# leejaehot/GaussianGrasper

Hardware: AMD Instinct MI355X
Metric: rendered views/sec (fwd+bwd) at 1M Gaussians, 1600x1200, 32-ch feature (higher is better)
Workload: dtype f32; 1 GPU; BASELINE config 4 per-GPU share: 1000000 Gaussians, 1600x1200, SH deg 4 rgb + 32-ch feature + depth + normal images per view (nerfstudio plugin route: the timed callable is FusedGaussianSplattingModel.get_outputs(camera) of gaussiangrasper_amd.plugin (the class train.sh loads, on stub.py's stand-ins for nerfstudio's base model and Cameras) — one fused rasterize operator per view), fwd+bwd, 8 views; route=plugin, deterministic_backward=False, python_gc=gc.freeze() after the warm-up (bench.freeze_gc), view_pipeline=backward of view k beside forward of view k + 1 on two streams, num_gaussians=1000000, feature_dim=32, n_visible=992125, parallelism=view-parallel x1, replicated Gaussians, grad_allreduce_bytes=472000000, grad_allreduce=per parameter, overlapped with the last view's backward

## Files before the change

gaussiangrasper_amd/csrc/blend2.hip:

```cpp
#include <type_traits>

#include "blend_launch.h"

#define GRP 4
#define KEEP(x) asm volatile("" ::"v"(x))

#include "blend_measure.h"
#define LIST_CAP 72

template <int NC = 1>
struct WaveListT {
    float4 a[LIST_CAP];
    float4 b[LIST_CAP];
    float4 c[LIST_CAP];
    float4 d[NC >= 2 ? LIST_CAP : 1];
    float4 e[NC >= 3 ? LIST_CAP : 1];
};

struct Seg2 {
    const float *colors;
    const float *background;
    float *out_img;
    int C2, nch2;
};
// ... 3 lines not shown
    return __builtin_amdgcn_mbcnt_hi((uint32_t)(m >> 32), __builtin_amdgcn_mbcnt_lo((uint32_t)m, 0u));
}

template <int CH, bool WIDE, bool REL = false, typename LIST = WaveList>
__device__ __forceinline__ int stage_chunk(LIST &L, int lane, int e, bool valid,
                                           const int g ,
                                           const GRec *__restrict__ rec,
                                           const float *__restrict__ colors, int C, int ch_off, int nch,
                                           float xlo, float xhi, float ylo, float yhi,
                                           const Seg2 *seg2 = nullptr) {
    const float4 ra = reinterpret_cast<const float4 *>(rec + g)[0];
    const float4 rb = reinterpret_cast<const float4 *>(rec + g)[1];
    const bool hit = valid && rec_hits_rect(ra, rb, xlo, xhi, ylo, yhi);
    const uint64_t m = __ballot(hit);
    const int cnt = __builtin_popcountll(m);
    const int pos = GRP + lane_prefix(m);
    if (hit) {
        const float posf = __builtin_bit_cast(float, REL ? lane : e + 1);
        float4 cc = make_float4(0.f, 0.f, 0.f, posf);
        float4 ra2 = ra;
        if (WIDE) {
            cc.x = __builtin_bit_cast(float, g);
            if (seg2) {
                const float *c2 = seg2->colors + (size_t)g * seg2->C2;
                const int n2 = seg2->nch2;
                L.d[pos] = make_float4(c2[0], n2 > 1 ? c2[1] : 0.f, n2 > 2 ? c2[2] : 0.f, n2 > 3 ? c2[3] : 0.f);
                L.e[pos] = make_float4(n2 > 4 ? c2[4] : 0.f, n2 > 5 ? c2[5] : 0.f, n2 > 6 ? c2[6] : 0.f,
                                       n2 > 7 ? c2[7] : 0.f);
            }
        } else {
            const float *col = colors + (size_t)g * C + ch_off;
            cc.x = col[0];
            if (CH > 1 && nch > 1) cc.y = col[1];
            if (CH > 2 && nch > 2) cc.z = col[2];
            if (CH > 3) {
                cc.w = nch > 3 ? col[3] : 0.f;
                float4 dd = make_float4(0.f, 0.f, 0.f, 0.f);
                if (nch > 4) dd.x = col[4];
                if (nch > 5) dd.y = col[5];
                if (nch > 6) dd.z = col[6];
                if (nch > 7) dd.w = col[7];
                L.d[pos] = dd;
                ra2.w = posf;
            }
        }
        L.a[pos] = ra2;
        L.b[pos] = make_float4(rb.x, rb.y, rb.z, __builtin_bit_cast(float, g));
        L.c[pos] = cc;
    }
    if (lane < 2 * GRP) {
        const int q = (lane < GRP) ? lane : (cnt + lane);
        L.a[q] = make_float4(0.f, 0.f, 0.f, 0.f);
        L.b[q] = make_float4(0.f, 0.f, 0.f, __builtin_bit_cast(float, -1));
        L.c[q] = make_float4(0.f, 0.f, 0.f, 0.f);
        if (CH > 3 && !WIDE) L.d[q] = make_float4(0.f, 0.f, 0.f, 0.f);
        if (WIDE && seg2) {
            L.d[q] = make_float4(0.f, 0.f, 0.f, 0.f);
            L.e[q] = make_float4(0.f, 0.f, 0.f, 0.f);
        }
    }
    __builtin_amdgcn_wave_barrier();
    return cnt;
}

#ifndef GG_FWD_WAVES
#define GG_FWD_WAVES 5
#endif
template <int CH, bool WIDE, bool FULL, bool EX = false, int FABL = 0, int NCB = 1>
__global__ __launch_bounds__(64 * GG_WPB_OTHER)
__attribute__((amdgpu_waves_per_eu((WIDE && EX && NCB == 1) ? GG_FWD_WAVES : (NCB == 2 ? (EX ? 4 : 3) : (NCB > 2 ? 2 : 1)))))
void blend2_fwd_kernel(
    int C, int ch_off, int nch, int img_h, int img_w, int tiles_x, int ntiles,
    const int32_t *__restrict__ ids, const int2 *__restrict__ bins, const GRec *__restrict__ rec,
    const float *__restrict__ colors, const float *__restrict__ background,
    float *__restrict__ out_img, float *__restrict__ final_T, int32_t *__restrict__ final_idx,
    int write_final, Seg2 seg2 = Seg2()) {
    constexpr bool N8 = !WIDE && CH > 3;
    static_assert(!EX || WIDE, "the second array rides on the wide kernel");
    static_assert(NCB == 1 || (WIDE && FULL), "several channel blocks: the full wide builds");
    typedef WaveListT<EX ? 3 : (N8 ? 2 : 1)> LIST;
    __shared__ LIST lists[GG_WPB_OTHER];
    int wave;
    const int tile = blend_tile_wave<GG_WPB_OTHER>(blockIdx.x, threadIdx.x, ntiles, wave);
    if (tile < 0) return;
    const int lane = threadIdx.x & 63;
    const int wslot = wave & (GG_WPB_OTHER - 1);
    LIST &L = lists[wslot];
    const int tx = tile % tiles_x, ty = tile / tiles_x;
    const int qx0 = tx * GG_BLOCK + (wave & 1) * 8, qy0 = ty * GG_BLOCK + (wave >> 1) * 8;
    const int j = qx0 + (lane & 7), i = qy0 + (lane >> 3);
    const bool inside = (i < img_h) && (j < img_w);
    const float px = (float)j, py = (float)i;
    const float xlo = (float)qx0, xhi = (float)(qx0 + 7), ylo = (float)qy0, yhi = (float)(qy0 + 7);
    const int2 range = bins[tile];

    STAMP_DECL;
    float T = 1.0f;
    int last = range.x;
    bool done = !inside;
    float acc[WIDE ? 1 : CH];
    float acc2[EX ? 8 : 1];
#pragma unroll
    for (int c = 0; c < (EX ? 8 : 1); ++c) acc2[c] = 0.0f;
    f32x16 acc0[NCB], acc1[NCB];
#pragma unroll
    for (int c = 0; c < (WIDE ? 1 : CH); ++c) acc[c] = 0.0f;
#pragma unroll
    for (int cb = 0; cb < NCB; ++cb)
#pragma unroll
        for (int r = 0; r < 16; ++r) acc0[cb][r] = acc1[cb][r] = 0.0f;
    const int wch = lane & 31, half = lane >> 5;
    const bool wch_ok = FULL || wch < nch;

    STAMP(0);
    for (int base = range.x; base < range.y; base += 64) {
        if (__ballot(!done) == 0ull) break;
        const int e = base + lane;
        const int g_cur = e < range.y ? ids[e] : 0;
        const int cnt = stage_chunk<CH, WIDE, false, LIST>(L, lane, e, e < range.y, g_cur, rec, colors, C,
                                                           ch_off, nch, xlo, xhi, ylo, yhi, EX ? &seg2 : nullptr);
        WALK_STAT(0, min(64, range.y - base));
        STAMP(1);
        STAMP_BATCH();
        constexpr int fabl = FABL;
        if (fabl >= 4) { KEEP(cnt); continue; }
        for (int k = 0; k < cnt; k += GRP) {
            if (k > 0 && __ballot(!done) == 0ull) break;
            WALK_STAT(1, min(GRP, cnt - k));
            constexpr bool LEANF = WIDE && (EX || NCB > 1);
            float4 A[GRP], B[GRP], Cc[GRP], Cd[GRP];
#pragma unroll
            for (int q = 0; q < GRP; ++q) {
                if (LEANF) continue;
                A[q] = L.a[GRP + k + q];
                B[q] = L.b[GRP + k + q];
                Cc[q] = L.c[GRP + k + q];
                if (N8) Cd[q] = L.d[GRP + k + q];
            }
            float colB[GRP / 2][NCB];
            if (WIDE) {
#pragma unroll
                for (int pr = 0; pr < GRP / 2; ++pr) {
                    const int gid = __builtin_bit_cast(int, L.c[GRP + k + 2 * pr + half].x);
#pragma unroll
                    for (int cb = 0; cb < NCB; ++cb)
                        colB[pr][cb] = (wch_ok && fabl < 2) ? colors[(size_t)gid * C + ch_off + 32 * cb + wch] : 0.0f;
                }
            }
            float alpha[GRP];
            bool pass[GRP];
#pragma unroll
            for (int q = 0; q < GRP; ++q) {
                if (LEANF) {
                    A[q] = L.a[GRP + k + q];
                    B[q] = L.b[GRP + k + q];
                }
                const float dx = A[q].x - px, dy = A[q].y - py;
                const float sigma = __builtin_fmaf(
                    0.5f, __builtin_fmaf(B[q].x * dx, dx, (B[q].z * dy) * dy), (B[q].y * dx) * dy);
                alpha[q] = fminf(GG_ALPHA_MAX_FWD, A[q].z * gg_expf_walk(-sigma));
                pass[q] = sigma >= 0.0f && !(alpha[q] < GG_ALPHA_MIN);
                if (LEANF && q == 1) __builtin_amdgcn_sched_barrier(0);
            }
            float vis[GRP];
#pragma unroll
            for (int q = 0; q < GRP; ++q) {
                const float next_T = T * (1.0f - alpha[q]);
                const bool live = pass[q] && !done;
                const bool stop = live && (next_T <= GG_T_EPS);
                const bool blend = live && !stop;
                vis[q] = blend ? alpha[q] * T : 0.0f;
#ifdef GG_WALK_STATS
                {
                    const unsigned long long bm = __ballot(blend), pm = __ballot(pass[q]), lm = __ballot(!done);
                    WALK_STAT(2, bm != 0ull);
                    WALK_STAT(3, __builtin_popcountll(lm));
                    WALK_STAT(4, __builtin_popcountll(pm));
                    WALK_STAT(5, __builtin_popcountll(bm));
                }
#endif
                T = blend ? next_T : T;
                last = blend ? __builtin_bit_cast(int, N8 ? A[q].w : (LEANF ? L.c[GRP + k + q].w : Cc[q].w)) : last;
                done = done || stop;
                if (EX && fabl < 3) {
                    const float4 xd = L.d[GRP + k + q], xe = L.e[GRP + k + q];
                    acc2[0] = __builtin_fmaf(xd.x, vis[q], acc2[0]);
                    acc2[EX ? 1 : 0] = __builtin_fmaf(xd.y, vis[q], acc2[EX ? 1 : 0]);
                    acc2[EX ? 2 : 0] = __builtin_fmaf(xd.z, vis[q], acc2[EX ? 2 : 0]);
                    acc2[EX ? 3 : 0] = __builtin_fmaf(xd.w, vis[q], acc2[EX ? 3 : 0]);
                    acc2[EX ? 4 : 0] = __builtin_fmaf(xe.x, vis[q], acc2[EX ? 4 : 0]);
                    acc2[EX ? 5 : 0] = __builtin_fmaf(xe.y, vis[q], acc2[EX ? 5 : 0]);
                    acc2[EX ? 6 : 0] = __builtin_fmaf(xe.z, vis[q], acc2[EX ? 6 : 0]);
                    acc2[EX ? 7 : 0] = __builtin_fmaf(xe.w, vis[q], acc2[EX ? 7 : 0]);
                }
                if (!WIDE) {
                    acc[0] = __builtin_fmaf(Cc[q].x, vis[q], acc[0]);
                    if (CH > 1) acc[CH > 1 ? 1 : 0] = __builtin_fmaf(Cc[q].y, vis[q], acc[CH > 1 ? 1 : 0]);
                    if (CH > 2) acc[CH > 2 ? 2 : 0] = __builtin_fmaf(Cc[q].z, vis[q], acc[CH > 2 ? 2 : 0]);
                    if (N8) {
                        acc[CH > 3 ? 3 : 0] = __builtin_fmaf(Cc[q].w, vis[q], acc[CH > 3 ? 3 : 0]);
                        acc[CH > 4 ? 4 : 0] = __builtin_fmaf(Cd[q].x, vis[q], acc[CH > 4 ? 4 : 0]);
                        acc[CH > 5 ? 5 : 0] = __builtin_fmaf(Cd[q].y, vis[q], acc[CH > 5 ? 5 : 0]);
                        acc[CH > 6 ? 6 : 0] = __builtin_fmaf(Cd[q].z, vis[q], acc[CH > 6 ? 6 : 0]);
                        acc[CH > 7 ? 7 : 0] = __builtin_fmaf(Cd[q].w, vis[q], acc[CH > 7 ? 7 : 0]);
                    }
                }
            }
            if (WIDE && fabl >= 1) {
#pragma unroll
                for (int q = 0; q < GRP; ++q) KEEP(vis[q]);
#pragma unroll
                for (int pr = 0; pr < GRP / 2; ++pr) KEEP(colB[pr][0]);
            } else if (WIDE) {
#pragma unroll
                for (int pr = 0; pr < GRP / 2; ++pr) {
                    auto r = __builtin_amdgcn_permlane32_swap(
                        __builtin_bit_cast(unsigned, vis[2 * pr]),
                        __builtin_bit_cast(unsigned, vis[2 * pr + 1]), false, false);
#pragma unroll
                    for (int cb = 0; cb < NCB; ++cb) {
                        acc0[cb] = __builtin_amdgcn_mfma_f32_32x32x2f32(__builtin_bit_cast(float, (unsigned)r[0]),
                                                                        colB[pr][cb], acc0[cb], 0, 0, 0);
                        acc1[cb] = __builtin_amdgcn_mfma_f32_32x32x2f32(__builtin_bit_cast(float, (unsigned)r[1]),
                                                                        colB[pr][cb], acc1[cb], 0, 0, 0);
                    }
                }
            }
        }
        __builtin_amdgcn_wave_barrier();
        STAMP(4);
    }
    STAMP(8);
    if (inside && write_final) {
        const size_t p = (size_t)i * img_w + j;
        final_T[p] = T;
        final_idx[p] = last;
    }
    if (EX && inside) {
        float *o2 = seg2.out_img + ((size_t)i * img_w + j) * seg2.C2;
#pragma unroll
        for (int c = 0; c < 8; ++c)
            if (c < seg2.nch2) o2[c] = __builtin_fmaf(T, seg2.background[c], acc2[EX ? c : 0]);
    }
    if (!WIDE) {
        if (inside) {
            float *o = out_img + ((size_t)i * img_w + j) * C + ch_off;
#pragma unroll
            for (int c = 0; c < CH; ++c)
                if (c < nch) o[c] = __builtin_fmaf(T, background[ch_off + c], acc[c]);
        }
    } else if (FULL && (C % 4 == 0) && (ch_off % 4 == 0) && ((reinterpret_cast<uintptr_t>(out_img) & 15) == 0)) {
        float *buf = reinterpret_cast<float *>(&L);
        const int chunk = lane & 7;
        __builtin_amdgcn_wave_barrier();
#pragma unroll
        for (int cb = 0; cb < NCB; ++cb) {
        const int ch_cb = ch_off + 32 * cb;
        const float4 bg4 = *reinterpret_cast<const float4 *>(background + ch_cb + 4 * chunk);
#pragma unroll
        for (int q4 = 0; q4 < 4; ++q4) {
#pragma unroll
            for (int rr = 0; rr < 8; ++rr) {
                const int r = 8 * (q4 & 1) + rr;
                const int pl = (rr & 3) + 8 * (rr >> 2) + 4 * half;
                buf[pl * 32 + wch] = (q4 >> 1) ? acc1[cb][r] : acc0[cb][r];
            }
            __builtin_amdgcn_wave_barrier();
#pragma unroll
            for (int t = 0; t < 2; ++t) {
                const int pl = (lane >> 3) + 8 * t;
                const float4 v = *reinterpret_cast<const float4 *>(buf + pl * 32 + 4 * chunk);
                const int pq = 16 * q4 + pl;
                const float Tp = __shfl(T, pq, 64);
                const int pj = qx0 + (pq & 7), pi = qy0 + (pq >> 3);
                if (pi < img_h && pj < img_w) {
                    typedef float f4v __attribute__((ext_vector_type(4)));
                    const f4v o = {__builtin_fmaf(Tp, bg4.x, v.x), __builtin_fmaf(Tp, bg4.y, v.y),
                                   __builtin_fmaf(Tp, bg4.z, v.z), __builtin_fmaf(Tp, bg4.w, v.w)};
                    f4v *dst = reinterpret_cast<f4v *>(out_img + ((size_t)pi * img_w + pj) * C + ch_cb + 4 * chunk);
                    *dst = o;
                }
            }
            __builtin_amdgcn_wave_barrier();
        }
        }
    } else {
        const float bgc = wch_ok ? background[ch_off + wch] : 0.0f;
#pragma unroll
        for (int blk = 0; blk < 2; ++blk)
#pragma unroll
            for (int r = 0; r < 16; ++r) {
                const int pq = 32 * blk + (r & 3) + 8 * (r >> 2) + 4 * half;
                const float Tp = __shfl(T, pq, 64);
                const int pj = qx0 + (pq & 7), pi = qy0 + (pq >> 3);
                if (pi < img_h && pj < img_w && wch_ok)
                    out_img[((size_t)pi * img_w + pj) * C + ch_off + wch] =
                        __builtin_fmaf(Tp, bgc, blk ? acc1[0][r] : acc0[0][r]);
            }
    }
    STAMP(7);
    STAMP_END();
}

#define FB_SLOTS 32
#define FB_QCAP 100
#ifndef GG_FB_WAVES
#define GG_FB_WAVES 3
#endif
struct __attribute__((aligned(16))) FwdQueue {
    float4 a[FB_QCAP];
    float4 b[FB_QCAP];
};
#define GG_VIS_SCALE 32768.0f
#define GG_VIS_UNSCALE (1.0f / 32768.0f)

__global__ __launch_bounds__(64) __attribute__((amdgpu_waves_per_eu(GG_FB_WAVES))) void blend2_fwd_batch_kernel(
    int C, int img_h, int img_w, int tiles_x, int ntiles, const int32_t *__restrict__ ids,
    const int2 *__restrict__ bins, const GRec *__restrict__ rec, const float *__restrict__ colors,
    const float *__restrict__ background, float *__restrict__ out_img, float *__restrict__ final_T,
    int32_t *__restrict__ final_idx, Seg2 seg2, unsigned bytes1, unsigned bytes2) {
    __shared__ FwdQueue s_q;
    __shared__ __attribute__((aligned(16))) float s_vis[64 * FB_SLOTS];
    int wave;
    const int tile = blend_tile_wave<1>(blockIdx.x, threadIdx.x, ntiles, wave);
    if (tile < 0) return;
    const int lane = threadIdx.x & 63;
    FwdQueue &Q = s_q;
    float *vis_w = s_vis;
    const int tx = tile % tiles_x, ty = tile / tiles_x;
    const int qx0 = tx * GG_BLOCK + (wave & 1) * 8, qy0 = ty * GG_BLOCK + (wave >> 1) * 8;
    const int j = qx0 + (lane & 7), i = qy0 + (lane >> 3);
    const bool inside = (i < img_h) && (j < img_w);
    const float px = (float)j, py = (float)i;
    const int2 range = bins[tile];
    const int sl = lane & 15, q4 = lane >> 4;

    float T = GG_VIS_SCALE;
    int last = range.x;
    bool done = !inside;
    bool alive = true;
    float csc[3];
#pragma unroll
    for (int nb = 0; nb < 3; ++nb) csc[nb] = pow2_scale(0.0f);
    f32x4 acc[4][3];
#pragma unroll
    for (int blk = 0; blk < 4; ++blk)
#pragma unroll
        for (int nb = 0; nb < 3; ++nb) acc[blk][nb] = f32x4{0.0f, 0.0f, 0.0f, 0.0f};
    const bool ch2_ok = sl < seg2.nch2;
    const __amdgpu_buffer_rsrc_t rs1 = __builtin_amdgcn_make_buffer_rsrc(const_cast<float *>(colors), 0, (int)bytes1, 0x00020000);
    const __amdgpu_buffer_rsrc_t rs2 = __builtin_amdgcn_make_buffer_rsrc(const_cast<float *>(seg2.colors), 0, (int)bytes2, 0x00020000);
    const unsigned rowb1 = 4u * (unsigned)C, rowb2 = 4u * (unsigned)seg2.C2;
    const unsigned lane_off1 = 4u * (unsigned)sl, lane_off2 = ch2_ok ? 4u * (unsigned)sl : 0u;

    auto run_batch = [&](const int base, const int n) {
        float cb[3][8];
#pragma unroll
        for (int t = 0; t < 8; ++t) {
            const int s_ = min(8 * q4 + t, n - 1);
            const unsigned gid = (unsigned)__builtin_bit_cast(int, Q.b[base + s_].w);
            const unsigned o1 = __umul24(gid, rowb1) + lane_off1;
            cb[0][t] = __builtin_bit_cast(float, __builtin_amdgcn_raw_buffer_load_b32(rs1, (int)o1, 0, 0));
            cb[1][t] = __builtin_bit_cast(float, __builtin_amdgcn_raw_buffer_load_b32(rs1, (int)o1 + 64, 0, 0));
            const unsigned o2 = __umul24(gid, rowb2) + lane_off2;
            const float c2v = __builtin_bit_cast(float, __builtin_amdgcn_raw_buffer_load_b32(rs2, (int)o2, 0, 0));
            cb[2][t] = ch2_ok ? c2v : 0.0f;
        }
        int nw = 0;
        for (int g = 0; g < n; g += GRP) {
            if (__ballot(!done) == 0ull) { alive = false; break; }
            float vis[GRP];
#pragma unroll
            for (int q = 0; q < GRP; ++q) {
                const float4 A = Q.a[base + g + q], B = Q.b[base + g + q];
                const float dx = A.x - px, dy = A.y - py;
                const float sigma = __builtin_fmaf(
                    0.5f, __builtin_fmaf(B.x * dx, dx, (B.z * dy) * dy), (B.y * dx) * dy);
                const float alpha = fminf(GG_ALPHA_MAX_FWD, A.z * gg_expf_walk(-sigma));
                const bool pass = sigma >= 0.0f && !(alpha < GG_ALPHA_MIN);
                const float next_T = T * (1.0f - alpha);
                const bool live = pass && !done;
                const bool stop = live && (next_T <= GG_T_EPS * GG_VIS_SCALE);
                const bool blend = live && !stop;
                vis[q] = blend ? alpha * T : 0.0f;
                T = blend ? next_T : T;
                last = blend ? __builtin_bit_cast(int, A.w) : last;
                done = done || stop;
                if (q == 1) __builtin_amdgcn_sched_barrier(0);
            }
            *reinterpret_cast<float4 *>(vis_w + lane * FB_SLOTS + ((((g >> 2) ^ lane) & 7) << 2)) =
                make_float4(vis[0], vis[1], vis[2], vis[3]);
            nw = g + GRP;
        }
        for (int g = nw; g < FB_SLOTS; g += GRP)
            *reinterpret_cast<float4 *>(vis_w + lane * FB_SLOTS + ((((g >> 2) ^ lane) & 7) << 2)) =
                make_float4(0.0f, 0.0f, 0.0f, 0.0f);
        __builtin_amdgcn_wave_barrier();
        h16x8 Bh[3], Bl[3];
        float fac[3];
        bool shrink = false;
#pragma unroll
        for (int nb = 0; nb < 3; ++nb) {
            float m = fmaxf(fmaxf(fabsf(cb[nb][0]), fabsf(cb[nb][1])), fabsf(cb[nb][2]));
            m = fmaxf(fmaxf(m, fabsf(cb[nb][3])), fabsf(cb[nb][4]));
            m = fmaxf(fmaxf(m, fabsf(cb[nb][5])), fmaxf(fabsf(cb[nb][6]), fabsf(cb[nb][7])));
            {
                auto r16 = __builtin_amdgcn_permlane16_swap(__builtin_bit_cast(unsigned, m), __builtin_bit_cast(unsigned, m), false, false);
                m = fmaxf(__builtin_bit_cast(float, (unsigned)r16[0]), __builtin_bit_cast(float, (unsigned)r16[1]));
                auto r32 = __builtin_amdgcn_permlane32_swap(__builtin_bit_cast(unsigned, m), __builtin_bit_cast(unsigned, m), false, false);
                m = fmaxf(__builtin_bit_cast(float, (unsigned)r32[0]), __builtin_bit_cast(float, (unsigned)r32[1]));
            }
            const float sb = fminf(csc[nb], pow2_scale(m));
            fac[nb] = sb * pow2_inv(csc[nb]);
            shrink = shrink || sb != csc[nb];
            csc[nb] = sb;
            unsigned h_[4], l_[4];
#pragma unroll
            for (int t = 0; t < 4; ++t) split2h(cb[nb][2 * t] * sb, cb[nb][2 * t + 1] * sb, h_[t], l_[t]);
            Bh[nb] = H8(h_[0], h_[1], h_[2], h_[3]);
            Bl[nb] = H8(l_[0], l_[1], l_[2], l_[3]);
        }
        if (__ballot(shrink) != 0ull) {
#pragma unroll
            for (int blk = 0; blk < 4; ++blk)
#pragma unroll
                for (int nb = 0; nb < 3; ++nb)
#pragma unroll
                    for (int r = 0; r < 4; ++r) acc[blk][nb][r] *= fac[nb];
        }
#pragma unroll
        for (int blk = 0; blk < 4; ++blk) {
            const int P = 16 * blk + sl;
            const float4 v0 = *reinterpret_cast<const float4 *>(vis_w + P * FB_SLOTS + ((((2 * q4) ^ P) & 7) << 2));
            const float4 v1 = *reinterpret_cast<const float4 *>(vis_w + P * FB_SLOTS + ((((2 * q4 + 1) ^ P) & 7) << 2));
            unsigned ah[4], al[4];
            split2h(v0.x, v0.y, ah[0], al[0]);
            split2h(v0.z, v0.w, ah[1], al[1]);
            split2h(v1.x, v1.y, ah[2], al[2]);
            split2h(v1.z, v1.w, ah[3], al[3]);
            const h16x8 Ah = H8(ah[0], ah[1], ah[2], ah[3]), Al = H8(al[0], al[1], al[2], al[3]);
#pragma unroll
            for (int nb = 0; nb < 3; ++nb) {
                acc[blk][nb] = __builtin_amdgcn_mfma_f32_16x16x32_f16(Al, Bl[nb], acc[blk][nb], 0, 0, 0);
                acc[blk][nb] = __builtin_amdgcn_mfma_f32_16x16x32_f16(Al, Bh[nb], acc[blk][nb], 0, 0, 0);
                acc[blk][nb] = __builtin_amdgcn_mfma_f32_16x16x32_f16(Ah, Bl[nb], acc[blk][nb], 0, 0, 0);
                acc[blk][nb] = __builtin_amdgcn_mfma_f32_16x16x32_f16(Ah, Bh[nb], acc[blk][nb], 0, 0, 0);
            }
        }
        __builtin_amdgcn_wave_barrier();
    };

    int qn = 0;
    int g_nxt = (range.x + lane < range.y) ? ids[range.x + lane] : 0;
    for (int cbase = range.x; cbase < range.y; cbase += 64) {
        if (__ballot(!done) == 0ull) { alive = false; break; }
        const int e = cbase + lane;
        const bool valid = e < range.y;
        const int g = g_nxt;
        g_nxt = (e + 64 < range.y) ? ids[e + 64] : 0;
        const float4 ra = reinterpret_cast<const float4 *>(rec + g)[0];
        const float4 rb = reinterpret_cast<const float4 *>(rec + g)[1];
        int qxl = qx0, qyl = qy0;
        asm volatile("" : "+s"(qxl), "+s"(qyl));
        const bool hit = valid && rec_hits_rect(ra, rb, (float)qxl, (float)(qxl + 7), (float)qyl, (float)(qyl + 7));
        const uint64_t m = __ballot(hit);
        if (hit) {
            const int pos = qn + lane_prefix(m);
            Q.a[pos] = make_float4(ra.x, ra.y, ra.z, __builtin_bit_cast(float, e + 1));
            Q.b[pos] = make_float4(rb.x, rb.y, rb.z, __builtin_bit_cast(float, g));
        }
        qn += __builtin_popcountll(m);
        __builtin_amdgcn_wave_barrier();
        int done_n = 0;
        while (qn - done_n >= FB_SLOTS && alive) {
            run_batch(done_n, FB_SLOTS);
            done_n += FB_SLOTS;
        }
        if (!alive) break;
        if (done_n > 0) {
            const int left = qn - done_n;
            if (lane < left) { const float4 ta = Q.a[done_n + lane]; __builtin_amdgcn_wave_barrier(); Q.a[lane] = ta; }
            __builtin_amdgcn_wave_barrier();
            if (lane < left) { const float4 tb = Q.b[done_n + lane]; __builtin_amdgcn_wave_barrier(); Q.b[lane] = tb; }
            qn = left;
            __builtin_amdgcn_wave_barrier();
        }
    }
    if (alive && qn > 0) {
        if (lane < GRP) {
            Q.a[qn + lane] = make_float4(0.f, 0.f, 0.f, 0.f);
            Q.b[qn + lane] = make_float4(0.f, 0.f, 0.f, Q.b[qn - 1].w);
        }
        __builtin_amdgcn_wave_barrier();
        run_batch(0, qn);
    }

    T *= GG_VIS_UNSCALE;
    if (inside) {
        const size_t p = (size_t)i * img_w + j;
        final_T[p] = T;
        final_idx[p] = last;
    }
#pragma unroll
    for (int nb = 0; nb < 3; ++nb) {
        const float un = pow2_inv(csc[nb]) * GG_VIS_UNSCALE;
#pragma unroll
        for (int blk = 0; blk < 4; ++blk)
#pragma unroll
            for (int r = 0; r < 4; ++r) acc[blk][nb][r] *= un;
    }
    __builtin_amdgcn_wave_barrier();
#pragma unroll
    for (int blk = 0; blk < 4; ++blk)
#pragma unroll
        for (int nb = 0; nb < 2; ++nb)
#pragma unroll
            for (int r = 0; r < 4; ++r) vis_w[(16 * blk + 4 * q4 + r) * 32 + 16 * nb + sl] = acc[blk][nb][r];
    __builtin_amdgcn_wave_barrier();
    {
        const int chunk = lane & 7;
        const float4 bg4 = *reinterpret_cast<const float4 *>(background + 4 * chunk);
#pragma unroll
        for (int t = 0; t < 8; ++t) {
            const int pq = (lane >> 3) + 8 * t;
            const float4 v = *reinterpret_cast<const float4 *>(vis_w + pq * 32 + 4 * chunk);
            const float Tp = __shfl(T, pq, 64);
            const int pj = qx0 + (pq & 7), pi = qy0 + (pq >> 3);
            if (pi < img_h && pj < img_w) {
                typedef float f4v __attribute__((ext_vector_type(4)));
                const f4v o = {__builtin_fmaf(Tp, bg4.x, v.x), __builtin_fmaf(Tp, bg4.y, v.y),
                               __builtin_fmaf(Tp, bg4.z, v.z), __builtin_fmaf(Tp, bg4.w, v.w)};
                *reinterpret_cast<f4v *>(out_img + ((size_t)pi * img_w + pj) * C + 4 * chunk) = o;
            }
        }
    }
    __builtin_amdgcn_wave_barrier();
    if (sl < 8) {
#pragma unroll
        for (int blk = 0; blk < 4; ++blk)
#pragma unroll
            for (int r = 0; r < 4; ++r) vis_w[(16 * blk + 4 * q4 + r) * 8 + sl] = acc[blk][2][r];
    }
    __builtin_amdgcn_wave_barrier();
    if (inside) {
        const float4 w0 = *reinterpret_cast<const float4 *>(vis_w + lane * 8);
        const float4 w1 = *reinterpret_cast<const float4 *>(vis_w + lane * 8 + 4);
        const float wv[8] = {w0.x, w0.y, w0.z, w0.w, w1.x, w1.y, w1.z, w1.w};
        float *o2 = seg2.out_img + ((size_t)i * img_w + j) * seg2.C2;
#pragma unroll
        for (int c = 0; c < 8; ++c)
            if (c < seg2.nch2) o2[c] = __builtin_fmaf(T, seg2.background[c], wv[c]);
    }
}

template <int CH, int ABL = 0, bool DET = false>
__global__ __launch_bounds__(64 * GG_WPB_OTHER) void blend2_bwd_narrow_kernel(
    int C, int ch_off, int nch, int img_h, int img_w, int tiles_x, int ntiles,
    const int32_t *__restrict__ ids, const int2 *__restrict__ bins, const GRec *__restrict__ rec,
    const float *__restrict__ colors, const float *__restrict__ background,
    const float *__restrict__ final_T, const int32_t *__restrict__ final_idx,
    const float *__restrict__ v_out, float *__restrict__ v_xy, float *__restrict__ v_conic,
    float *__restrict__ v_colors, float *__restrict__ v_opacity, int gstride, int cstride,
    DetSlab det = DetSlab()) {
    constexpr int K = CH + 6;
    constexpr int KB = GRP * K;
    using R = Red6<KB>;
    constexpr bool N8 = CH > 3;
    typedef WaveListT<N8 ? 2 : 1> LIST;
    __shared__ LIST lists[GG_WPB_OTHER];

    int wave;
    const int tile = blend_tile_wave<GG_WPB_OTHER>(blockIdx.x, threadIdx.x, ntiles, wave);
    if (tile < 0) return;
    const int lane = threadIdx.x & 63;
    const int wslot = wave & (GG_WPB_OTHER - 1);
    LIST &L = lists[wslot];
    const int tx = tile % tiles_x, ty = tile / tiles_x;
    const int qx0 = tx * GG_BLOCK + (wave & 1) * 8, qy0 = ty * GG_BLOCK + (wave >> 1) * 8;
    const int j = qx0 + (lane & 7), i = qy0 + (lane >> 3);
    const bool inside = (i < img_h) && (j < img_w);
    const float px = (float)j, py = (float)i;
    const float xlo = (float)qx0, xhi = (float)(qx0 + 7), ylo = (float)qy0, yhi = (float)(qy0 + 7);
    const int2 range = bins[tile];
    const size_t p = inside ? ((size_t)i * img_w + j) : 0;

    const float T_final = inside ? final_T[p] : 1.0f;
    const int fin = inside ? min(max(final_idx[p], range.x), range.y) : range.x;
    float T = T_final;
    float vo[CH];
    float W;
    {
        float Bsum = 0.0f;
#pragma unroll
        for (int c = 0; c < CH; ++c) {
            const bool chan = !N8 || c < nch;
            vo[c] = (inside && chan) ? v_out[p * C + ch_off + c] : 0.0f;
            if (chan) Bsum = __builtin_fmaf(background[ch_off + c], vo[c], Bsum);
        }
        W = T_final * Bsum;
    }
    int hi = fin;
    for (int off = 32; off > 0; off >>= 1) hi = max(hi, __shfl_xor(hi, off, 64));
    hi = __builtin_amdgcn_readfirstlane(hi);

    bool owner;
    const int myvar = R::var(lane, owner);
    const int my_q = myvar / K, my_k = myvar - my_q * K;
    float *my_base;
    int my_stride;
    if (my_k < CH) {
        my_base = v_colors + ch_off + my_k;
        my_stride = cstride ? cstride : C;
        owner = owner && (!N8 || my_k < nch);
    }
    else if (my_k < CH + 2) { my_base = v_xy + (my_k - CH); my_stride = gstride ? gstride : 2; }
    else if (my_k < CH + 5) { my_base = v_conic + (my_k - CH - 2); my_stride = gstride ? gstride : 3; }
    else { my_base = v_opacity; my_stride = gstride ? gstride : 1; }

    int g_nxt = (N8 && hi > range.x && hi - 64 + lane >= range.x) ? ids[hi - 64 + lane] : 0;
    for (int top = hi; top > range.x; top -= 64) {
        const int e = top - 64 + lane;
        const bool valid = e >= range.x;
        int g_cur;
        if (N8) {
            g_cur = g_nxt;
            g_nxt = (top - 64 > range.x && e - 64 >= range.x) ? ids[e - 64] : 0;
        } else {
            g_cur = valid ? ids[e] : 0;
        }
        const int cnt = stage_chunk<CH, false, true, LIST>(L, lane, e, valid, g_cur, rec, colors, C, ch_off,
                                                           N8 ? nch : CH, xlo, xhi, ylo, yhi);
        const int fin_rel = fin - (top - 64);
        if (ABL >= 4) { KEEP(cnt); continue; }
        for (int kk = GRP + cnt - 1; kk >= GRP; kk -= GRP) {
            float4 A[GRP], B[GRP], Cc[GRP], Cd[GRP];
#pragma unroll
            for (int q = 0; q < GRP; ++q) {
                A[q] = L.a[kk - q];
                B[q] = L.b[kk - q];
                Cc[q] = L.c[kk - q];
                if (N8) Cd[q] = L.d[kk - q];
            }
            float vis[GRP], alpha[GRP], dxs[GRP], dys[GRP];
            bool pass[GRP];
#pragma unroll
            for (int q = 0; q < GRP; ++q) {
                const float dx = A[q].x - px, dy = A[q].y - py;
                dxs[q] = dx;
                dys[q] = dy;
                const float sigma = __builtin_fmaf(
                    0.5f, __builtin_fmaf(B[q].x * dx, dx, (B[q].z * dy) * dy), (B[q].y * dx) * dy);
                vis[q] = gg_expf_walk(-sigma);
                alpha[q] = fminf(GG_ALPHA_MAX_BWD, A[q].z * vis[q]);
                pass[q] = (__builtin_bit_cast(int, N8 ? A[q].w : Cc[q].w) < fin_rel) && sigma >= 0.0f &&
                          !(alpha[q] < GG_ALPHA_MIN);
            }
            if (__ballot(pass[0] || pass[1] || pass[2] || pass[3]) == 0ull) continue;
            if (ABL >= 3) {
#pragma unroll
                for (int q = 0; q < GRP; ++q) { KEEP(vis[q]); KEEP(alpha[q]); KEEP((int)pass[q]); }
                continue;
            }

            float part[KB];
#pragma unroll
            for (int q = 0; q < GRP; ++q) {
                const float ra_ = __builtin_amdgcn_rcpf(1.0f - alpha[q]);
                const float Tn = T * ra_;
                const float fac = pass[q] ? alpha[q] * Tn : 0.0f;
                float D = Cc[q].x * vo[0];
                if (CH > 1) D = __builtin_fmaf(Cc[q].y, vo[CH > 1 ? 1 : 0], D);
                if (CH > 2) D = __builtin_fmaf(Cc[q].z, vo[CH > 2 ? 2 : 0], D);
                if (N8) {
                    D = __builtin_fmaf(Cc[q].w, vo[CH > 3 ? 3 : 0], D);
                    D = __builtin_fmaf(Cd[q].x, vo[CH > 4 ? 4 : 0], D);
                    D = __builtin_fmaf(Cd[q].y, vo[CH > 5 ? 5 : 0], D);
                    D = __builtin_fmaf(Cd[q].z, vo[CH > 6 ? 6 : 0], D);
                    D = __builtin_fmaf(Cd[q].w, vo[CH > 7 ? 7 : 0], D);
                }
#pragma unroll
                for (int c = 0; c < CH; ++c) part[q * K + c] = fac * vo[c];
                const float v_alpha = pass[q] ? (Tn * D - ra_ * W) : 0.0f;
                W = pass[q] ? __builtin_fmaf(D, fac, W) : W;
                T = pass[q] ? Tn : T;
                const float v_sigma = pass[q] ? (-A[q].z * vis[q]) * v_alpha : 0.0f;
                const float dx = dxs[q], dy = dys[q];
                float *pg = part + q * K + CH;
                pg[0] = v_sigma * (B[q].x * dx + B[q].y * dy);
                pg[1] = v_sigma * (B[q].y * dx + B[q].z * dy);
                const float hs = 0.5f * v_sigma;
                pg[2] = (hs * dx) * dx;
                pg[3] = (hs * dx) * dy;
                pg[4] = (hs * dy) * dy;
                pg[5] = pass[q] ? vis[q] * v_alpha : 0.0f;
            }
            if (ABL >= 2) {
#pragma unroll
                for (int v = 0; v < KB; ++v) KEEP(part[v]);
                continue;
            }
            const float mine = R::run(part, lane);
            const int my_gid = __builtin_bit_cast(int, L.b[kk - my_q].w);
            if (ABL >= 1) { KEEP(mine); KEEP(my_gid); continue; }
            if (DET) {
                const int pos = __builtin_bit_cast(int, N8 ? L.a[kk - my_q].w : L.c[kk - my_q].w);
                const size_t e = (size_t)(top - 64 + pos);
                if (owner && my_gid >= 0)
                    det.p[(e * 4 + wave) * det.ks + (my_k < CH ? det.coff + my_k : det.goff + (my_k - CH))] = mine;
                continue;
            }
            if (owner && my_gid >= 0 && mine != 0.0f) atomicAdd(my_base + (size_t)my_gid * my_stride, mine);
        }
        __builtin_amdgcn_wave_barrier();
    }
}

#define B2_SLOTS 32
#ifndef GG_S16_STRIDE
#define GG_S16_STRIDE 65
#endif
#define FIDX(slot, pix) ((slot) * FS + (pix))

#define GG_FAC_SCALE 32768.0f
#define GG_FAC_UNSCALE (1.0f / 32768.0f)
#ifndef GG_S16_WAVES
#define GG_S16_WAVES 4
#endif

#define BQ_CAP 92

template <int CAP>
struct __attribute__((aligned(16))) WaveQueueT {
    float4 a[CAP];
    float4 b[CAP];
};
typedef WaveQueueT<BQ_CAP> WaveQueue;

struct Seg2B {
    const float *colors;
    const float *background;
    const float *v_out[3];
    int vo_w[3];
    float *v_colors;
    int C2, nch2, cs2;
};

template <bool FULL, int ABL = 0, int CHD = 32, bool DET = false, bool EX = false, bool S16 = false, bool MG = false>
__global__ __launch_bounds__(64 * GG_WPB_WIDE_BWD) __attribute__((amdgpu_waves_per_eu(S16 ? GG_S16_WAVES : 3))) void blend2_bwd_wide_kernel(
    int C, int ch_off, int nch, int img_h, int img_w, int tiles_x, int ntiles,
    const int32_t *__restrict__ ids, const int2 *__restrict__ bins, const GRec *__restrict__ rec,
    const float *__restrict__ colors, const float *__restrict__ background,
    const float *__restrict__ final_T, const int32_t *__restrict__ final_idx,
    const float *__restrict__ v_out, float *__restrict__ v_xy, float *__restrict__ v_conic,
    float *__restrict__ v_colors, float *__restrict__ v_opacity, int gstride, int cstride,
    DetSlab det = DetSlab(), Seg2B seg2 = Seg2B()) {
    static_assert(!MG || (S16 && EX), "merged record flush: the 16-slot pair build");
    static_assert(!EX || (FULL && CHD == 32 && !DET), "the second array rides on the full 32-channel build");
    static_assert(!S16 || (FULL && CHD == 32 && !DET && ABL == 0), "S16: the full 32-channel build");
    constexpr int NSLOT = S16 ? 16 : B2_SLOTS;
    constexpr int CH = CHD;
    constexpr int KS = CHD / 2;
    constexpr int KG = 6;
    constexpr int KB = GRP * KG;
    constexpr bool REREAD = S16;
    using R = Red6<KB>;
    typedef WaveQueueT<BQ_CAP> QUEUE;
    __shared__ QUEUE queues[GG_WPB_WIDE_BWD];
    constexpr int FS = S16 ? GG_S16_STRIDE : 65;
    __shared__ float s_fac[GG_WPB_WIDE_BWD][NSLOT * FS];
    __shared__ int s_slote[GG_WPB_WIDE_BWD][DET ? B2_SLOTS : 1];
    __shared__ __attribute__((aligned(16))) float s_vt[GG_WPB_WIDE_BWD][EX ? 64 * 8 + 8 : 4];
    __shared__ float s_geo[GG_WPB_WIDE_BWD][MG ? 16 * 8 : 1];

    int wave;
    const int tile = blend_tile_wave<GG_WPB_WIDE_BWD>(blockIdx.x, threadIdx.x, ntiles, wave);
    if (tile < 0) return;
    const int lane = threadIdx.x & 63;
    const int wslot = wave & (GG_WPB_WIDE_BWD - 1);
    float *vt = s_vt[wslot];
    QUEUE &Q = queues[wslot];
    float *fac_w = s_fac[wslot];
    float *geo_w = s_geo[wslot];
    int *slote = s_slote[wslot];
    const int tx = tile % tiles_x, ty = tile / tiles_x;
    const int qx0 = tx * GG_BLOCK + (wave & 1) * 8, qy0 = ty * GG_BLOCK + (wave >> 1) * 8;
    const int j = qx0 + (lane & 7), i = qy0 + (lane >> 3);
    const bool inside = (i < img_h) && (j < img_w);
    const float px = (float)j, py = (float)i;
    const int2 range = bins[tile];
    const size_t p = inside ? ((size_t)i * img_w + j) : 0;

    STAMP_DECL;
    const float T_final = inside ? final_T[p] : 1.0f;
    const int fin = inside ? min(max(final_idx[p], range.x), range.y) : range.x;
    float T = T_final;
    float W;
    const int wch = lane & 31, half = lane >> 5;
    const bool wch_ok = FULL || wch < nch;
    const bool tile_lds = FULL && CH == 32 && (C % 4 == 0) && (ch_off % 4 == 0) &&
                      ((reinterpret_cast<uintptr_t>(v_out) & 15) == 0);
    float voa_keep[2][S16 ? 1 : KS], vob_keep[S16 ? 1 : 32];
    float va16[S16 ? 4 : 1][S16 ? 8 : 1], vb16[S16 ? 16 : 1][S16 ? 2 : 1];
    constexpr bool F2 = S16 && EX;
    unsigned vah[S16 ? 4 : 1][S16 ? 4 : 1], val[S16 ? 4 : 1][S16 ? 4 : 1];
    unsigned vbh[S16 ? 2 : 1][S16 ? 2 : 1][S16 ? 4 : 1], vbl[S16 ? 2 : 1][S16 ? 2 : 1][S16 ? 4 : 1];
    float sw = 1.0f, inv_sw = 1.0f, inv_scf[2] = {1.0f, 1.0f};
    float Bsum = 0.0f;
    auto wave_hi = [&]() {
        int h = fin;
        for (int off = 32; off > 0; off >>= 1) h = max(h, __shfl_xor(h, off, 64));
        return __builtin_amdgcn_readfirstlane(h);
    };
    auto load_id = [&](int top_) {
        const int e_ = top_ - 64 + lane;
        return (top_ > range.x && e_ >= range.x) ? ids[e_] : 0;
    };
    int hi, g_first;
    float4 ra_p = make_float4(0.f, 0.f, 0.f, 0.f), rb_p = ra_p;
    if (S16) {
        hi = wave_hi();
        g_first = load_id(hi);
        const int sl = lane & 15, q4 = lane >> 4;
#pragma unroll
        for (int hh = 0; hh < 2; ++hh) {
            float4 rowv[4];
#pragma unroll
            for (int rr = 0; rr < 4; ++rr) {
                const int pi = qy0 + 4 * hh + rr, pj = qx0 + (lane >> 3);
                rowv[rr] = (pi < img_h && pj < img_w)
                               ? *reinterpret_cast<const float4 *>(v_out + ((size_t)pi * img_w + pj) * C + ch_off + 4 * (lane & 7))
                               : make_float4(0.f, 0.f, 0.f, 0.f);
            }
            __builtin_amdgcn_wave_barrier();
#pragma unroll
            for (int rr = 0; rr < 4; ++rr) {
// ... 839 lines not shown
```

Measured before the change: 635.5 views/s.

## Halve forward blend batch to 16 slots and raise waves per EU to four

```diff
diff --git a/gaussiangrasper_amd/csrc/blend2.hip b/gaussiangrasper_amd/csrc/blend2.hip
--- a/gaussiangrasper_amd/csrc/blend2.hip
+++ b/gaussiangrasper_amd/csrc/blend2.hip
@@ -329,10 +329,13 @@
     STAMP_END();
 }
 
-#define FB_SLOTS 32
-#define FB_QCAP 100
+#define FB_SLOTS 16
+#define FB_QCAP 84
 #ifndef GG_FB_WAVES
-#define GG_FB_WAVES 3
+#define GG_FB_WAVES 4
+#endif
+#ifndef GG_FB_ALWAYS_EXCHANGE
+#define GG_FB_ALWAYS_EXCHANGE 0
 #endif
 struct __attribute__((aligned(16))) FwdQueue {
     float4 a[FB_QCAP];
@@ -348,6 +351,10 @@
     int32_t *__restrict__ final_idx, Seg2 seg2, unsigned bytes1, unsigned bytes2) {
     __shared__ FwdQueue s_q;
     __shared__ __attribute__((aligned(16))) float s_vis[64 * FB_SLOTS];
+#ifdef GG_FB_LDS_PAD
+    __shared__ char s_pad[GG_FB_LDS_PAD];
+    asm volatile("" ::"v"(&s_pad[threadIdx.x]));
+#endif
     int wave;
     const int tile = blend_tile_wave<1>(blockIdx.x, threadIdx.x, ntiles, wave);
     if (tile < 0) return;
@@ -381,10 +388,10 @@
     const unsigned lane_off1 = 4u * (unsigned)sl, lane_off2 = ch2_ok ? 4u * (unsigned)sl : 0u;
 
     auto run_batch = [&](const int base, const int n) {
-        float cb[3][8];
-#pragma unroll
-        for (int t = 0; t < 8; ++t) {
-            const int s_ = min(8 * q4 + t, n - 1);
+        float cb[3][4];
+#pragma unroll
+        for (int t = 0; t < 4; ++t) {
+            const int s_ = min(4 * q4 + t, n - 1);
             const unsigned gid = (unsigned)__builtin_bit_cast(int, Q.b[base + s_].w);
             const unsigned o1 = __umul24(gid, rowb1) + lane_off1;
             cb[0][t] = __builtin_bit_cast(float, __builtin_amdgcn_raw_buffer_load_b32(rs1, (int)o1, 0, 0));
@@ -415,64 +422,52 @@
                 done = done || stop;
                 if (q == 1) __builtin_amdgcn_sched_barrier(0);
             }
-            *reinterpret_cast<float4 *>(vis_w + lane * FB_SLOTS + ((((g >> 2) ^ lane) & 7) << 2)) =
+            *reinterpret_cast<float4 *>(vis_w + lane * FB_SLOTS + ((((g >> 2) ^ (lane >> 1)) & 3) << 2)) =
                 make_float4(vis[0], vis[1], vis[2], vis[3]);
             nw = g + GRP;
         }
         for (int g = nw; g < FB_SLOTS; g += GRP)
-            *reinterpret_cast<float4 *>(vis_w + lane * FB_SLOTS + ((((g >> 2) ^ lane) & 7) << 2)) =
+            *reinterpret_cast<float4 *>(vis_w + lane * FB_SLOTS + ((((g >> 2) ^ (lane >> 1)) & 3) << 2)) =
                 make_float4(0.0f, 0.0f, 0.0f, 0.0f);
         __builtin_amdgcn_wave_barrier();
         h16x8 Bh[3], Bl[3];
-        float fac[3];
-        bool shrink = false;
 #pragma unroll
         for (int nb = 0; nb < 3; ++nb) {
-            float m = fmaxf(fmaxf(fabsf(cb[nb][0]), fabsf(cb[nb][1])), fabsf(cb[nb][2]));
-            m = fmaxf(fmaxf(m, fabsf(cb[nb][3])), fabsf(cb[nb][4]));
-            m = fmaxf(fmaxf(m, fabsf(cb[nb][5])), fmaxf(fabsf(cb[nb][6]), fabsf(cb[nb][7])));
-            {
+            float m = fmaxf(fmaxf(fabsf(cb[nb][0]), fabsf(cb[nb][1])), fmaxf(fabsf(cb[nb][2]), fabsf(cb[nb][3])));
+            if (GG_FB_ALWAYS_EXCHANGE || __ballot(pow2_scale(m) < csc[nb]) != 0ull) {
                 auto r16 = __builtin_amdgcn_permlane16_swap(__builtin_bit_cast(unsigned, m), __builtin_bit_cast(unsigned, m), false, false);
                 m = fmaxf(__builtin_bit_cast(float, (unsigned)r16[0]), __builtin_bit_cast(float, (unsigned)r16[1]));
                 auto r32 = __builtin_amdgcn_permlane32_swap(__builtin_bit_cast(unsigned, m), __builtin_bit_cast(unsigned, m), false, false);
                 m = fmaxf(__builtin_bit_cast(float, (unsigned)r32[0]), __builtin_bit_cast(float, (unsigned)r32[1]));
-            }
-            const float sb = fminf(csc[nb], pow2_scale(m));
-            fac[nb] = sb * pow2_inv(csc[nb]);
-            shrink = shrink || sb != csc[nb];
-            csc[nb] = sb;
-            unsigned h_[4], l_[4];
-#pragma unroll
-            for (int t = 0; t < 4; ++t) split2h(cb[nb][2 * t] * sb, cb[nb][2 * t + 1] * sb, h_[t], l_[t]);
-            Bh[nb] = H8(h_[0], h_[1], h_[2], h_[3]);
-            Bl[nb] = H8(l_[0], l_[1], l_[2], l_[3]);
-        }
-        if (__ballot(shrink) != 0ull) {
-#pragma unroll
-            for (int blk = 0; blk < 4; ++blk)
-#pragma unroll
-                for (int nb = 0; nb < 3; ++nb)
-#pragma unroll
-                    for (int r = 0; r < 4; ++r) acc[blk][nb][r] *= fac[nb];
+                const float sb = fminf(csc[nb], pow2_scale(m));
+                if (__ballot(sb != csc[nb]) != 0ull) {
+                    const float fac = sb * pow2_inv(csc[nb]);
+#pragma unroll
+                    for (int blk = 0; blk < 4; ++blk)
+#pragma unroll
+                        for (int r = 0; r < 4; ++r) acc[blk][nb][r] *= fac;
+                }
+                csc[nb] = sb;
+            }
+            const float sb = csc[nb];
+            unsigned h0, l0, h1, l1;
+            split2h(cb[nb][0] * sb, cb[nb][1] * sb, h0, l0);
+            split2h(cb[nb][2] * sb, cb[nb][3] * sb, h1, l1);
+            Bh[nb] = H8(h0, h1, h0, h1);
+            Bl[nb] = H8(l0, l1, l0, l1);
         }
 #pragma unroll
         for (int blk = 0; blk < 4; ++blk) {
             const int P = 16 * blk + sl;
-            const float4 v0 = *reinterpret_cast<const float4 *>(vis_w + P * FB_SLOTS + ((((2 * q4) ^ P) & 7) << 2));
-            const float4 v1 = *reinterpret_cast<const float4 *>(vis_w + P * FB_SLOTS + ((((2 * q4 + 1) ^ P) & 7) << 2));
-            unsigned ah[4], al[4];
-            split2h(v0.x, v0.y, ah[0], al[0]);
-            split2h(v0.z, v0.w, ah[1], al[1]);
-            split2h(v1.x, v1.y, ah[2], al[2]);
-            split2h(v1.z, v1.w, ah[3], al[3]);
-            const h16x8 Ah = H8(ah[0], ah[1], ah[2], ah[3]), Al = H8(al[0], al[1], al[2], al[3]);
-#pragma unroll
-            for (int nb = 0; nb < 3; ++nb) {
-                acc[blk][nb] = __builtin_amdgcn_mfma_f32_16x16x32_f16(Al, Bl[nb], acc[blk][nb], 0, 0, 0);
-                acc[blk][nb] = __builtin_amdgcn_mfma_f32_16x16x32_f16(Al, Bh[nb], acc[blk][nb], 0, 0, 0);
-                acc[blk][nb] = __builtin_amdgcn_mfma_f32_16x16x32_f16(Ah, Bl[nb], acc[blk][nb], 0, 0, 0);
-                acc[blk][nb] = __builtin_amdgcn_mfma_f32_16x16x32_f16(Ah, Bh[nb], acc[blk][nb], 0, 0, 0);
-            }
+            const float4 v = *reinterpret_cast<const float4 *>(vis_w + P * FB_SLOTS + (((q4 ^ (sl >> 1)) & 3) << 2));
+            unsigned ah0, al0, ah1, al1;
+            split2h(v.x, v.y, ah0, al0);
+            split2h(v.z, v.w, ah1, al1);
+            const h16x8 A = H8(ah0, ah1, al0, al1);
+#pragma unroll
+            for (int nb = 0; nb < 3; ++nb) acc[blk][nb] = __builtin_amdgcn_mfma_f32_16x16x32_f16(A, Bl[nb], acc[blk][nb], 0, 0, 0);
+#pragma unroll
+            for (int nb = 0; nb < 3; ++nb) acc[blk][nb] = __builtin_amdgcn_mfma_f32_16x16x32_f16(A, Bh[nb], acc[blk][nb], 0, 0, 0);
         }
         __builtin_amdgcn_wave_barrier();
     };
@@ -536,28 +531,31 @@
 #pragma unroll
             for (int r = 0; r < 4; ++r) acc[blk][nb][r] *= un;
     }
-    __builtin_amdgcn_wave_barrier();
-#pragma unroll
-    for (int blk = 0; blk < 4; ++blk)
-#pragma unroll
-        for (int nb = 0; nb < 2; ++nb)
-#pragma unroll
-            for (int r = 0; r < 4; ++r) vis_w[(16 * blk + 4 * q4 + r) * 32 + 16 * nb + sl] = acc[blk][nb][r];
-    __builtin_amdgcn_wave_barrier();
     {
         const int chunk = lane & 7;
         const float4 bg4 = *reinterpret_cast<const float4 *>(background + 4 * chunk);
 #pragma unroll
-        for (int t = 0; t < 8; ++t) {
-            const int pq = (lane >> 3) + 8 * t;
-            const float4 v = *reinterpret_cast<const float4 *>(vis_w + pq * 32 + 4 * chunk);
-            const float Tp = __shfl(T, pq, 64);
-            const int pj = qx0 + (pq & 7), pi = qy0 + (pq >> 3);
-            if (pi < img_h && pj < img_w) {
-                typedef float f4v __attribute__((ext_vector_type(4)));
-                const f4v o = {__builtin_fmaf(Tp, bg4.x, v.x), __builtin_fmaf(Tp, bg4.y, v.y),
-                               __builtin_fmaf(Tp, bg4.z, v.z), __builtin_fmaf(Tp, bg4.w, v.w)};
-                *reinterpret_cast<f4v *>(out_img + ((size_t)pi * img_w + pj) * C + 4 * chunk) = o;
+        for (int half = 0; half < 2; ++half) {
+            __builtin_amdgcn_wave_barrier();
+#pragma unroll
+            for (int b2 = 0; b2 < 2; ++b2)
+#pragma unroll
+                for (int nb = 0; nb < 2; ++nb)
+#pragma unroll
+                    for (int r = 0; r < 4; ++r) vis_w[(16 * b2 + 4 * q4 + r) * 32 + 16 * nb + sl] = acc[2 * half + b2][nb][r];
+            __builtin_amdgcn_wave_barrier();
+#pragma unroll
+            for (int t = 0; t < 4; ++t) {
+                const int pl = (lane >> 3) + 8 * t, pq = 32 * half + pl;
+                const float4 v = *reinterpret_cast<const float4 *>(vis_w + pl * 32 + 4 * chunk);
+                const float Tp = __shfl(T, pq, 64);
+                const int pj = qx0 + (pq & 7), pi = qy0 + (pq >> 3);
+                if (pi < img_h && pj < img_w) {
+                    typedef float f4v __attribute__((ext_vector_type(4)));
+                    const f4v o = {__builtin_fmaf(Tp, bg4.x, v.x), __builtin_fmaf(Tp, bg4.y, v.y),
+                                   __builtin_fmaf(Tp, bg4.z, v.z), __builtin_fmaf(Tp, bg4.w, v.w)};
+                    *reinterpret_cast<f4v *>(out_img + ((size_t)pi * img_w + pj) * C + 4 * chunk) = o;
+                }
             }
         }
     }
```

Result: faster. 645.3 views/s, median of 6 (+1.5%).
